# ZenGo-X/zk-paillier

Measured on AMD Instinct MI355X. Metric: RangeProofNi proofs/sec + verifies/sec, n=2048, batch=4096 per GPU (value = verifies/sec; proofs/sec in prove.value), higher is better.
Workload: dtype u32 (29-bit limbs, u64 accumulate)

## Files before the change

zk-paillier_amd/csrc/kernels_basen.hpp:

```cpp
#pragma once
#include "kernels_modexp.hpp"

#define ZKP_UNROLL_STR(x) #x
#define ZKP_UNROLL_(n) _Pragma(ZKP_UNROLL_STR(unroll n))
#define ZKP_UNROLL(n) ZKP_UNROLL_(n)
#ifndef ZKP_BN_ROW_UNROLL
#if ZKP_W == 9
#define ZKP_BN_ROW_UNROLL 8
#else
#define ZKP_BN_ROW_UNROLL 1
#endif
#endif
#ifndef ZKP_BN_ASM
#define ZKP_BN_ASM (ZKP_W == 36)
#endif
namespace zkp {
template <int G> constexpr bool BN_ASM_G = ZKP_BN_ASM && W == 36 && (G == 2 || G == 4);

template <int G> struct BnConst {
  static constexpr int L = Geo<G>::L;
  static constexpr int OFF_MT = 0, OFF_C3 = L, OFF_RRA = 2 * L, OFF_RRB = 3 * L, OFF_N = 4 * L, OFF_R2N = 5 * L, OFF_ONE = 6 * L, OFF_R1A = 7 * L, OFF_R1B = 8 * L, OFF_NI = 9 * L, OFF_OK = 9 * L + 1;
  static constexpr int WORDS = 9 * L + 4;
  static constexpr int STRIDE = WORDS + 2 * L;
};
// ... 532 lines not shown
  store_limbs_global<G>(tab, X, g.gl);
  store_limbs_global<G>(tab + L, Y, g.gl);
  bn_stage<G>(g, g.A(), X);
  bn_stage<G>(g, g.B(), Y);
  const int msb = 31 - __clz(CAP);
#pragma unroll 1
  for (int b = msb - 1; b >= 0; b--) {
    bn_square<G>(g, X);
    if ((CAP >> b) & 1) {
      uint32_t A2[W], B2[W];
      bn_product<G>(g, A2, B2, tab, tab + L);
      bn_stage<G>(g, g.A(), A2);
      bn_stage<G>(g, g.B(), B2);
#pragma unroll
      for (int k = 0; k < W; k++) X[k] = A2[k];
    }
  }
  lds_load_block(Y, g.B() + g.gl * BLK);
  store_limbs_global<G>(out + BC::OFF_RRA, X, g.gl);
  store_limbs_global<G>(out + BC::OFF_RRB, Y, g.gl);
  store_limbs_global<G>(out + BC::OFF_R1A, OA, g.gl);
  store_limbs_global<G>(out + BC::OFF_R1B, OB, g.gl);
  if (g.gl == 0) {
    out[BC::OFF_OK] = ok ? 1u : 0u;
    if (!ok) atomicAnd(all_ok, 0u);
  }
  if (tag && up_tag && gid == 0 && g.gl == 0) {
    tag[1] = up_tag[5];
    __threadfence();
    tag[0] = (ok && up_tag[0] == SETUP_TAG_MAGIC) ? SETUP_TAG_MAGIC : 0u;
  }
}

template <int GS>
__global__ void __launch_bounds__(256, ZKP_WPE) k_expected(EncArgs a, uint32_t* __restrict__ expected, const uint32_t* __restrict__ bn_ok) {
  using CL = ConstLayout<GS>;
  using LL = LdsLayout<GS>;
  if (!*bn_ok) return;
  extern __shared__ __align__(16) uint32_t lds_raw[];
  Grp<GS> g;
  grp_init<GS>(g, lds_raw);
  const int kw = a.n_bits / 32;
  const uint64_t count = a.count_ptr ? (uint64_t)*a.count_ptr : a.count;
  const uint64_t stride = (uint64_t)gridDim.x * LL::GROUPS_PER_BLOCK;
  const uint64_t rounds = (count + stride - 1) / stride;
  const uint32_t* cst = a.consts;
  load_modulus_consts<GS>(g, cst);
  for (uint64_t rd = 0; rd < rounds; rd++) {
    const uint64_t idx = rd * stride + (uint64_t)blockIdx.x * LL::GROUPS_PER_BLOCK + (threadIdx.x / GS);
    const bool live = idx < count;
    const uint64_t item = live ? idx : count - 1;
    uint64_t b;
    bool mask_row;
    const uint32_t* pexp;
    if (a.mode == 2) { b = item; mask_row = a.cipher_x != nullptr; pexp = a.c1 + item * 2 * kw; }
    else {
      b = a.item_proof[item];
      const uint32_t rw = a.item_row[item];
      const uint64_t row = b * a.ef + (rw >> 1);
      mask_row = a.resp_kind[row] != 0;
      const bool use_c1 = mask_row ? (a.resp_j[row] == 1) : !(rw & 1);
      pexp = (use_c1 ? a.c1 : a.c2) + row * 2 * kw;
    }
    if (a.const_stride) {
      const uint64_t i0 = (a.mode == 0 && a.half && item >= a.half) ? item - a.half : item;
      cst = a.consts + (a.mode == 1 ? b : i0 / a.items_per_key) * a.const_stride;
      load_modulus_consts<GS>(g, cst);
    }
    const bool valid = cst[CL::OFF_ST] == 0;
    uint32_t A[W], R[W], Y[W];
    load_value<GS>(g, A, pexp, valid ? 2 * kw : 0);
    stage_const<GS>(g, cst + CL::OFF_R2);
    mm<GS>(g, R, A);
    {
      uint32_t t[W];
      load_value<GS>(g, t, a.cipher_x + b * 2 * kw, (mask_row && valid) ? 2 * kw : 0);
      if (!mask_row && valid && g.gl == 0) t[0] = 1;
      stageB<GS>(g, t);
    }
    mm<GS>(g, Y, R);
    stage_const<GS>(g, cst + CL::OFF_R2);
    mm<GS>(g, R, Y);
    stage_one<GS>(g);
    mm<GS>(g, Y, R);
    canonical_words<GS>(g, Y, cst + CL::OFF_N);
    if (live && mask_row) for (int w = g.gl; w < 2 * kw; w += GS) expected[item * 2 * kw + w] = g.words()[w];
  }
}

struct BnItem {
  const uint32_t* pm; const uint32_t* pr; const uint32_t* pexp; uint32_t* pout;
  uint64_t b; int mw, rw; bool mask_row;
};
__device__ __forceinline__ BnItem bn_item(const EncArgs& a, uint64_t item, const uint32_t* expected) {
  BnItem it{};
  const int kw = a.n_bits / 32;
  it.mw = kw; it.rw = kw;
  if (a.mode == 0) {
    const bool second = a.half && item >= a.half;
    const uint64_t i = second ? item - a.half : item;
    it.mw = a.m_words < 0 ? 0 : (a.m_words ? a.m_words : kw);
    it.rw = a.r_words ? a.r_words : kw;
    it.pm = (second ? a.m2 : a.m) + i * it.mw;
    it.pr = (second ? a.r2 : a.r) + i * it.rw;
    it.pout = (second ? a.out2 : a.out) + i * 2 * kw;
  } else if (a.mode == 2) {
    it.b = item;
    it.pm = a.m + item * kw;
    it.pr = a.r + item * kw;
    it.mask_row = a.cipher_x != nullptr;
    it.pexp = it.mask_row ? expected + item * 2 * kw : a.c1 + item * 2 * kw;
  } else {
    it.b = a.item_proof[item];
    const uint32_t rw = a.item_row[item];
    const uint64_t row = it.b * a.ef + (rw >> 1);
    it.mask_row = a.resp_kind[row] != 0;
    const bool second = (rw & 1) != 0;
    it.pm = (second ? a.resp_w2 : a.resp_w1) + row * kw;
    it.pr = (second ? a.resp_r2 : a.resp_r1) + row * kw;
// ... 568 lines not shown
```

zk-paillier_amd/csrc/kernels_modexp.hpp:

```cpp
#pragma once
#include "../../include/zkp_hip.h"
#include "bigint29.hpp"

namespace zkp {

#ifndef ZKP_WIN
#define ZKP_WIN 5
#endif
#ifndef ZKP_SWIN
#define ZKP_SWIN 6
#endif
#ifndef ZKP_WIN_KEY
#define ZKP_WIN_KEY 6
#endif
constexpr int WIN = ZKP_WIN;
constexpr int WIN_KEY = ZKP_WIN_KEY;
constexpr int SWIN = ZKP_SWIN;
constexpr int TABS = 1 << (SWIN - 1);
constexpr int cmax(int a, int b) { return a > b ? a : b; }
constexpr int TAB = cmax(cmax(1 << WIN, 1 << WIN_KEY), TABS);
static_assert(TABS <= 32 && WIN >= 2 && WIN <= 7 && WIN_KEY >= 2 && WIN_KEY <= 7, "window widths");

template <int G> struct ConstLayout {
  static constexpr int L = Geo<G>::L;
// ... 70 lines not shown
}

template <int G, class LL> __device__ __forceinline__ void mm(const Grp<G, LL>& g, uint32_t (&R)[W], const uint32_t (&A)[W]) {
  montmul<G, false, true>(R, A, g.B(), g.N, g.n1, g.gl);
}
template <int G, class LL> __device__ __forceinline__ void fetch_words(const Grp<G, LL>& g, uint32_t* dst, const uint32_t* src, int nwords) {
  constexpr int NW = LL::NW;
  wave_lds_fence();
  for (int w = g.gl; w < NW + 8; w += G) dst[w] = (w < nwords) ? src[w] : 0u;
  wave_lds_fence();
}

template <int G, class LL> __device__ __forceinline__ void load_value(const Grp<G, LL>& g, uint32_t (&v)[W], const uint32_t* src, int nwords) {
  fetch_words<G>(g, g.words(), src, nwords);
  limbs_from_words(v, g.words(), g.gl);
}

template <int G, class LL> __device__ __forceinline__ void canonical_limbs(const Grp<G, LL>& g, uint32_t (&x)[W]) {
  normalize_exact<G>(x, g.gl);
  bool eq = true;
#pragma unroll
  for (int k = 0; k < W; k++) eq = eq && (x[k] == g.N[k]);
  const unsigned long long m = __ballot(eq);
  const int lane = threadIdx.x & 63;
  const unsigned long long gm = (G == 64) ? ~0ull : (((1ull << G) - 1) << (lane & ~(G - 1)));
  if ((m & gm) == gm) {
#pragma unroll
    for (int k = 0; k < W; k++) x[k] = 0;
  }
}
template <int G, class LL> __device__ __forceinline__ void canonical_words(const Grp<G, LL>& g, uint32_t (&x)[W], const uint32_t* ) {
  canonical_limbs<G>(g, x);
  words_from_limbs<G, LL::NW>(g.words(), g.scr(), x, g.gl);
}


template <int G, bool SAFE, bool TWO = false, int SCHED_FENCE = 0, class LL> __device__ __forceinline__ void mmo_ip(const Grp<G, LL>& g, const uint32_t (&NT)[W], uint32_t (&X)[W]) {
  if constexpr (TWO) montmul2<G>(X, X, g.B(), NT, g.gl);
  else montmul<G, true, SAFE, SCHED_FENCE>(X, X, g.B(), NT, 1u, g.gl);
}
#ifndef ZKP_SQR
#define ZKP_SQR 1
#endif

template <bool SAFE, bool TWO> constexpr bool ladder_squares() { return ZKP_SQR && !SAFE; }
template <int G, bool TWO = false, class LL> __device__ __forceinline__ void msq_ip(const Grp<G, LL>& g, const uint32_t (&NT)[W], uint32_t (&X)[W]) {
  if constexpr (TWO) montsqr2<G>(X, g.B(), NT, g.gl);
  else montsqr<G>(X, g.B(), NT, g.gl);
}

template <int G> __device__ __forceinline__ int wave_exponent_bits(const uint32_t* lw, int exp_bits) {
  int top = (exp_bits >> 5) - 1;
  while (top > 0 && lw[top] == 0) top--;
  int bl = lw[top] ? 32 * top + 32 - __clz(lw[top]) : 0;
#pragma unroll
  for (int off = 32; off >= G && off >= 1; off >>= 1) { const int o = __shfl_xor(bl, off); bl = o > bl ? o : bl; }
  return __builtin_amdgcn_readfirstlane(bl);
}

template <int G, bool SAFE, bool TWO = false, int WIN = zkp::WIN, class LL>
__device__ __forceinline__ void powm_fixed(const Grp<G, LL>& g, uint32_t (&X)[W], int exp_bits, uint32_t* tab, const uint32_t* cst,
                                           const uint32_t* __restrict__ ew ) {
  using CL = ConstLayout<G>;
  constexpr int L = Geo<G>::L;
  constexpr int TABF = 1 << WIN;
  uint32_t NT[W];
// ... 668 lines not shown
```

zk-paillier_amd/csrc/kernels_proofs.hpp:

```cpp
#pragma once
#include "kernels_modexp.hpp"
#include "kernels_gcd.hpp"
#include "sha256_dev.hpp"

namespace zkp {

__device__ __forceinline__ int cmp_words(const uint32_t* a, const uint32_t* b, int n) {
  for (int i = n - 1; i >= 0; i--) {
    const uint32_t x = a[i], y = b[i];
    if (x != y) return x > y ? 1 : -1;
  }
  return 0;
}

__device__ __forceinline__ int challenge_bit(const uint8_t* e, uint32_t i) { return (e[i >> 3] >> (7 - (i & 7))) & 1; }

struct RangeHashArgs {
  const uint32_t* n; uint64_t n_stride;
  const uint32_t* c1; const uint32_t* c2; const uint32_t* range;
  uint32_t kw, ef; uint64_t batch;
  uint8_t* e;
  uint8_t* e_len;
  uint32_t* third;
  uint32_t* two_thirds;
// ... 243 lines not shown
  const uint8_t* db = reinterpret_cast<const uint8_t*>(s.row);
  int lead = 0;
  while (lead < 31 && db[lead] == 0) lead++;
  uint8_t* e = a.e + b * 32;
  for (int i = 0; i < 32; i++) e[i] = (i + lead < 32) ? db[i + lead] : 0;
  const int elen = 32 - lead;
  a.e_len[b] = (uint8_t)elen;
  a.verdict[b] = ((uint32_t)elen * 8 >= a.ef) ? a.ok_value : (uint8_t)ZKP_VERDICT_MALFORMED;
  if (!a.range) return;
  const uint32_t* rg = a.range + b * a.kw;
  uint32_t* t1 = a.third + b * a.kw;
  uint32_t* t2 = a.two_thirds + b * a.kw;
  uint64_t rem = 0;
  for (int w = (int)a.kw - 1; w >= 0; w--) {
    const uint64_t cur = (rem << 32) | rg[w];
    t1[w] = (uint32_t)(cur / 3);
    rem = cur % 3;
  }
  uint32_t carry = 0;
  for (uint32_t w = 0; w < a.kw; w++) { const uint32_t v = t1[w]; t2[w] = (v << 1) | carry; carry = v >> 31; }
}

#ifndef ZKP_TEMPLATE_KERNELS_ONLY
__global__ void __launch_bounds__(64) k_range_hash_wave(RangeHashArgs a) { range_hash_wave_body(a, (int)threadIdx.x, blockIdx.x); }
#endif

struct VerifyPlanArgs {
  const uint8_t* e; const uint8_t* resp_kind;
  const uint32_t* resp_w1; const uint32_t* resp_w2;
  const uint32_t* third; const uint32_t* two_thirds;
  uint32_t kw, ef; uint64_t batch;
  uint8_t* verdict;
  uint32_t* item_proof; uint32_t* item_row; unsigned long long* counter;
};

#ifndef ZKP_TEMPLATE_KERNELS_ONLY
__global__ void __launch_bounds__(256) k_verify_plan(VerifyPlanArgs a) {
  const uint64_t t = (uint64_t)blockIdx.x * 256 + threadIdx.x;
  const bool in = t < a.batch * a.ef;
  uint32_t nitems = 0;
  uint64_t b = 0; uint32_t i = 0;
  if (in && !a.e) {
    b = t / a.ef; i = (uint32_t)(t % a.ef);
    const int kind = a.resp_kind[t];
    nitems = kind == ZKP_RESP_OPEN ? 2 : kind == ZKP_RESP_MASK ? 1 : 0;
  } else if (in) {
    b = t / a.ef; i = (uint32_t)(t % a.ef);
    if (a.verdict[b] != ZKP_VERDICT_MALFORMED) {
      const int ei = challenge_bit(a.e + b * 32, i);
      const int kind = a.resp_kind[t];
      const uint32_t* T1 = a.third + b * a.kw;
      const uint32_t* T2 = a.two_thirds + b * a.kw;
      const uint32_t* w1 = a.resp_w1 + t * a.kw;
      if (!ei && kind == ZKP_RESP_OPEN) {
        const uint32_t* w2 = a.resp_w2 + t * a.kw;
        const int w1_T1 = cmp_words(w1, T1, a.kw), w2_T1 = cmp_words(w2, T1, a.kw);
        const bool flag = (w2_T1 < 0 && w1_T1 > 0 && cmp_words(w1, T2, a.kw) < 0) ||
                          (w1_T1 < 0 && w2_T1 > 0 && cmp_words(w2, T2, a.kw) < 0);
        if (!flag) a.verdict[b] = ZKP_VERDICT_REJECT;
        nitems = 2;
      } else if (ei && kind == ZKP_RESP_MASK) {
        if (cmp_words(w1, T1, a.kw) < 0 || cmp_words(w1, T2, a.kw) > 0) a.verdict[b] = ZKP_VERDICT_REJECT;
        nitems = 1;
      } else {
        a.verdict[b] = ZKP_VERDICT_REJECT;
      }
    }
  }
  if (!a.item_proof) return;
  const unsigned long long m2 = __ballot(nitems == 2), m1 = __ballot(nitems == 1);
  const int lane = threadIdx.x & 63;
  const unsigned long long lt = (1ull << lane) - 1;
  const uint32_t before = 2 * __popcll(m2 & lt) + __popcll(m1 & lt);
  const uint32_t total = 2 * __popcll(m2) + __popcll(m1);
  unsigned long long base = 0;
  if (lane == 0 && total) base = atomicAdd(a.counter, (unsigned long long)total);
  base = __shfl(base, 0);
  for (uint32_t k = 0; k < nitems; k++) {
    a.item_proof[base + before + k] = (uint32_t)b;
    a.item_row[base + before + k] = (i << 1) | k;
  }
}
#endif

struct VerdictMergeArgs {
  uint8_t* verdict; const uint8_t* enc_verdict; const uint8_t* e; const uint8_t* resp_kind; uint32_t ef; uint64_t batch;
};
#ifndef ZKP_TEMPLATE_KERNELS_ONLY
__global__ void __launch_bounds__(256) k_verdict_merge(VerdictMergeArgs a) {
  const uint64_t b = (uint64_t)blockIdx.x * 256 + threadIdx.x;
  if (b >= a.batch) return;
  const uint8_t v = a.verdict[b], ev = a.enc_verdict[b];
  if (v == ZKP_VERDICT_MALFORMED || ev == ZKP_VERDICT_ACCEPT) return;
  if (ev == ZKP_VERDICT_REJECT) { a.verdict[b] = ZKP_VERDICT_REJECT; return; }
  bool any = false;
  for (uint32_t i = 0; i < a.ef; i++) {
    const int ei = challenge_bit(a.e + b * 32, i), kind = a.resp_kind[b * a.ef + i];
    any = any || (!ei && kind == ZKP_RESP_OPEN) || (ei && kind == ZKP_RESP_MASK);
  }
  if (any) a.verdict[b] = ZKP_VERDICT_MALFORMED;
}
#endif

struct ResponseArgs {
  const uint32_t* consts; uint64_t const_stride;
  const uint32_t* x; const uint32_t* r;
  const uint32_t* w1; const uint32_t* w2; const uint32_t* r1; const uint32_t* r2;
  const uint8_t* e; const uint32_t* third; const uint32_t* two_thirds;
  uint8_t* resp_kind; uint8_t* resp_j; uint32_t* resp_w1; uint32_t* resp_r1; uint32_t* resp_w2; uint32_t* resp_r2;
  uint8_t* status;
  uint32_t kw, ef; uint64_t batch;
};

template <int G>
// ... 456 lines not shown
```

zk-paillier_amd/csrc/zkp_api.hip:

```cpp
#include <hip/hip_runtime.h>
#include <dlfcn.h>

#include <algorithm>
#include <cstdio>
#include <cstdlib>
#include <new>
#include <cstring>
#include <exception>
#include <mutex>
#include <string>
#include <thread>
#include <type_traits>
#include <vector>

#include "../../include/zkp_hip.h"
#include "../../include/zkp_hip_diag.h"
#include "kernels_modexp.hpp"
#include "kernels_proofs.hpp"
#include "kernels_inv.hpp"
#include "kernels_serde.hpp"
#include "kernels_serde_write.hpp"
#include "kernels_serde_scan.hpp"
#include "kernels_sample.hpp"
#include "kernels_coprime.hpp"
#if ZKP_W == 36 || ZKP_W == 18 || ZKP_W == 9
#define ZKP_HAS_BASEN 1
#include "kernels_basen.hpp"
#ifndef ZKP_R2L5_ITEMS_PER_CU
#define ZKP_R2L5_ITEMS_PER_CU 1ull
#endif
#include "kernels_basen_r2l.hpp"
#else
#define ZKP_HAS_BASEN 0
#endif

using namespace zkp;

struct DevBuf {
  void* p = nullptr;
  size_t cap = 0;
  uint32_t* tag = nullptr;
  uint64_t gen = 0, tag_gen = 0;
};

struct StageBlock { void* p; size_t cap; };

enum ScratchSlot : int {
  S_E = 0,
  S_ELEN = 1,
  S_T1 = 2, S_T2 = 3,
  S_IPROOF = 4, S_IROW = 5, S_COUNTER = 6,
  S_STATUS = 7,
  S_MGF = 8, S_PRIMES = 9,
  S_DLOG_E = 10,
  S_TMP1 = 11, S_TMP2 = 12, S_TMP3 = 13,
  S_SCHED = 15,
  S_TMP4 = 16, S_TMP5 = 17,
  S_WORK_COUNTER = 18,
  S_ENCV = 19,
  S_MP_NN = 20, S_MP_INVST = 21,
  S_MP_T0 = 22,
  S_MP_END = 32,
  S_CM_SUM = 34, S_CM_FLAGS = 35,
  S_CM_T0 = 36,
  S_CM_END = 44,
  S_SAMPLE_THIRD = 44, S_SAMPLE_META = 45, S_SAMPLE_STATUS = 46,
  S_RESIDUE = 47,
  S_COUNT = 48
};
static_assert(S_MP_T0 + 9 < S_MP_END && S_MP_END <= S_CM_SUM && S_CM_T0 + 7 < S_CM_END && S_CM_END <= S_SAMPLE_THIRD && S_RESIDUE < S_COUNT,
              "scratch slot runs overlap");

struct zkp_ctx {
  std::vector<StageBlock> stage_free;
  std::vector<std::pair<void*, size_t>> last_wiped;
  uint32_t* setup_flag = nullptr;
  uint32_t* setup_flag_host = nullptr;
  int device = 0;
  hipStream_t stream = nullptr;
  bool owns_stream = true;
  int cus = 0;
  const struct LatEngine* eng[2] = {nullptr, nullptr};
  zkp_ctx* eng_ctx[2] = {nullptr, nullptr};
  const struct LatEngine* lat = nullptr;
  zkp_ctx* lat_ctx = nullptr;
  int geometry = 0;
  int last_geometry = 0;
  hipStream_t side = nullptr;
  hipEvent_t ev_fork = nullptr, ev_join = nullptr;
  bool side_busy = false;
  hipStream_t copy = nullptr;
  std::vector<hipEvent_t> ev_pipe;
  bool copy_busy = false;
  int last_host_blocks = 0;
  uint64_t scan_fast = 0, scan_fallback = 0;
  hipEvent_t ev_scan[5] = {nullptr, nullptr, nullptr, nullptr, nullptr};
  int scan_phases = 0;
  zkp_ctx* split_ctx = nullptr;
  hipStream_t split_stream = nullptr;
  hipEvent_t ev_split[2] = {nullptr, nullptr};
  int split_calls = 1;
  int last_split = 0;
  int key_cache = 1;
  int host_chunks = -1;
  std::string err;
  DevBuf consts, consts2, table, scratch[S_COUNT];
  DevBuf bn_ncst, bn_consts, bn_table, bn_expected, bn_raw, bn_left;
  int enc_form = ZKP_ENC_FORM_AUTO;
  int bn_occ[2][2] = {{0, 0}, {0, 0}};
  int bn_last_g = 0;
  bool bn_last_per_key = false;
  bool bn_last_r2l = false;
  int bn_r2l_lanes = 0;
  int bn_last_r2l_lanes = 0;
  int bn_r2l = 1;
  const RangeHashArgs* fuse_hash = nullptr;
  bool fuse_hash_taken = false;
  int fuse_hash_on = 1;
  int grid_expected = 1;
  DevBuf bn_flag;
  bool timing = false;
  std::vector<std::pair<hipEvent_t, hipEvent_t>> ev;
  size_t ev_used = 0;
  uint64_t timed_launches = 0, timed_modexps = 0;
  static constexpr size_t PINNED_SLOTS = 4096;
  unsigned long long* pinned_counts = nullptr;
  size_t pinned_used = 0;
};

#define HIPCHK(ctx, call)                                                                         \
  do {                                                                                            \
    hipError_t e_ = (call);                                                                       \
    if (e_ != hipSuccess) {                                                                       \
      (ctx)->err = std::string(#call) + ": " + hipGetErrorString(e_);                             \
      return e_ == hipErrorOutOfMemory ? ZKP_ENOMEM : ZKP_EDEVICE;                                \
    }                                                                                             \
  } while (0)

static int32_t zkp_caught(zkp_ctx* c, int32_t st, const char* what) noexcept {
  if (c) { try { c->err = what; } catch (...) {} }
// ... 390 lines not shown
  HIPCHK(c, hipEventCreateWithFlags(&c->ev_fork, hipEventDisableTiming));
  HIPCHK(c, hipEventCreateWithFlags(&c->ev_join, hipEventDisableTiming));
  HIPCHK(c, hipStreamCreateWithFlags(&c->side, hipStreamNonBlocking));
  return ZKP_OK;
}

template <int G, class K> static int32_t table_for(zkp_ctx* c, K kernel, uint64_t items, unsigned* blocks_out) {
  using LL = LdsLayout<G>;
  const uint64_t need = (items + LL::GROUPS_PER_BLOCK - 1) / LL::GROUPS_PER_BLOCK;
  const unsigned blocks = (unsigned)std::max<uint64_t>(1, std::min<uint64_t>(need, (uint64_t)resident_blocks<G>(c, kernel)));
  *blocks_out = blocks;
  return ensure(c, c->table, (size_t)blocks * LL::GROUPS_PER_BLOCK * TAB * Geo<G>::L * sizeof(uint32_t));
}

constexpr bool PAIR_LADDER_BUILD = ZKP_W <= 9;
template <int G> static bool pair_ladder(const zkp_ctx* c, uint64_t items) {
  if (c->enc_form == ZKP_ENC_FORM_ALWAYS) return false;
  if constexpr (PAIR_LADDER_BUILD && 2 * G <= 64) return items * 2 * G <= 4ull * (uint64_t)c->cus * 64;
  (void)c; (void)items;
  return false;
}

#if ZKP_HAS_BASEN
constexpr int BN_GA = 72 / W, BN_GB = 144 / W;
#ifdef ZKP_SPLIT_TU
extern template __global__ void zkp::k_enc_basen<BN_GA>(EncArgs, const uint32_t*, uint32_t*, uint32_t*);
extern template __global__ void zkp::k_enc_basen<BN_GB>(EncArgs, const uint32_t*, uint32_t*, uint32_t*);
extern template __global__ void zkp::k_enc_basen_keys<BN_GA>(EncArgs, const uint32_t*, const uint32_t*, uint32_t*, uint32_t*);
extern template __global__ void zkp::k_enc_basen_keys<BN_GB>(EncArgs, const uint32_t*, const uint32_t*, uint32_t*, uint32_t*);
extern template __global__ void zkp::k_basen_finish<BN_GA>(EncArgs, const uint32_t*, const uint32_t*, int, const uint32_t*, const uint32_t*, const uint32_t*);
extern template __global__ void zkp::k_basen_finish<BN_GB>(EncArgs, const uint32_t*, const uint32_t*, int, const uint32_t*, const uint32_t*, const uint32_t*);
extern template __global__ void zkp::k_setup_basen<BN_GA>(const uint32_t*, uint32_t*, uint64_t, uint32_t*, const uint32_t*, uint32_t*);
extern template __global__ void zkp::k_setup_basen<BN_GB>(const uint32_t*, uint32_t*, uint64_t, uint32_t*, const uint32_t*, uint32_t*);
extern template __global__ void zkp::k_expected<2 * BN_GA>(EncArgs, uint32_t*, const uint32_t*);
extern template __global__ void zkp::k_expected<2 * BN_GB>(EncArgs, uint32_t*, const uint32_t*);
extern template __global__ void zkp::k_diag_basen<BN_GA>(const uint32_t*, int, const uint32_t*, const uint32_t*, const uint32_t*, const uint32_t*, uint32_t*, uint32_t*);
extern template __global__ void zkp::k_diag_basen<BN_GB>(const uint32_t*, int, const uint32_t*, const uint32_t*, const uint32_t*, const uint32_t*, uint32_t*, uint32_t*);
#endif
constexpr size_t BASEN_DIAG_LDS = 4096;
static int enc_form_from_env() {
  const char* e = std::getenv("ZKP_BASEN");
  if (e && e[0] == '0') return ZKP_ENC_FORM_N2;
  if (e && e[0] == 's') return ZKP_ENC_FORM_SHARED;
  if (e && e[0] == 'a') return ZKP_ENC_FORM_ALWAYS;
  return ZKP_ENC_FORM_AUTO;
}
template <int G> static int32_t basen_prepare(zkp_ctx* c, const uint32_t* n, uint64_t n_stride, uint64_t nkeys, uint32_t n_bits) {
  int32_t st = run_setup<G>(c, n, n_stride, (int)(n_bits / 32), 0, nkeys, c->bn_ncst);
  if (st) return st;
  if ((st = ensure(c, c->bn_consts, (size_t)(nkeys + 1) * BnConst<G>::STRIDE * sizeof(uint32_t)))) return st;
  HIPCHK(c, hipMemsetAsync((char*)c->bn_consts.p + (size_t)nkeys * BnConst<G>::STRIDE * sizeof(uint32_t), 0, BnConst<G>::STRIDE * sizeof(uint32_t), c->stream));
  if ((st = ensure(c, c->bn_flag, 64))) return st;
  HIPCHK(c, hipMemsetD32Async((hipDeviceptr_t)c->bn_flag.p, 1, 2, c->stream));
  constexpr unsigned GPB = 64 / G;
  uint32_t* tag = nullptr;
  if ((st = setup_tag(c, c->bn_consts, nkeys, &tag))) return st;
  hipLaunchKernelGGL(k_setup_basen<G>, dim3((unsigned)((nkeys + GPB - 1) / GPB)), dim3(64), GPB * BN_SETUP_LDS_WORDS * sizeof(uint32_t), c->stream,
                     (const uint32_t*)c->bn_ncst.p, (uint32_t*)c->bn_consts.p, nkeys, (uint32_t*)c->bn_flag.p, tag ? (const uint32_t*)c->bn_ncst.tag : nullptr, tag);
  HIPCHK(c, hipGetLastError());
  return ZKP_OK;
}
static bool r2l_one_per_simd(const zkp_ctx* c, uint64_t count, bool listed, uint64_t hashes) {
  const uint64_t simds = 4ull * (uint64_t)c->cus;
  const uint64_t expect = (listed && c->grid_expected) ? expected_items(count) : count;
  return hashes < simds && expect + hashes <= simds;
}
template <int GS> static bool launch_basen(zkp_ctx* c, const EncArgs& a_in, EncArgs* rest) {
  if constexpr (GS != 2 * BN_GA && GS != 2 * BN_GB) { (void)c; (void)a_in; (void)rest; return false; }
// ... 24 lines not shown
    }
    auto give_up = [&]() { c->err.clear(); *rest = a_in; return false; };
    if (basen_prepare<G>(c, a.n, a.n_stride, nkeys, (uint32_t)a.n_bits)) return give_up();
    int& per_cu = c->bn_occ[per_key ? 1 : 0][G == BN_GB ? 1 : 0];
    if (!per_cu) {
      const hipError_t e = per_key ? hipOccupancyMaxActiveBlocksPerMultiprocessor(&per_cu, k_enc_basen_keys<G>, 256, BL::BYTES_PER_BLOCK)
                                   : hipOccupancyMaxActiveBlocksPerMultiprocessor(&per_cu, k_enc_basen<G>, 256, BL::BYTES_PER_BLOCK);
      if (e != hipSuccess || per_cu < 1) per_cu = 1;
    }
    const uint64_t need = (a.count + BL::GROUPS_PER_BLOCK - 1) / BL::GROUPS_PER_BLOCK;
    uint64_t grid = std::min<uint64_t>(need, (uint64_t)per_cu * c->cus);
    if (a.count_ptr && a.mode == 1 && c->grid_expected) {
      const uint64_t need_e = (expected_items(a.count) + BL::GROUPS_PER_BLOCK - 1) / BL::GROUPS_PER_BLOCK;
      const uint64_t per_cu_e = (need_e + (uint64_t)c->cus - 1) / (uint64_t)c->cus;
      grid = std::min<uint64_t>(grid, per_cu_e * (uint64_t)c->cus);
    }
    const unsigned blocks = (unsigned)std::max<uint64_t>(1, grid);
    const size_t entries = per_key ? BN_KEYS_TAB_ENTRIES : BN_TAB_ENTRIES;
    if (!r2l_launch && ensure(c, c->bn_table, (size_t)blocks * BL::GROUPS_PER_BLOCK * entries * 2 * Geo<G>::L * sizeof(uint32_t))) return give_up();
    if (ensure(c, c->bn_raw, (size_t)a.count * 2 * Geo<G>::L * sizeof(uint32_t))) return give_up();
    const uint32_t* ok = per_key ? (const uint32_t*)c->bn_flag.p + 1 : (const uint32_t*)c->bn_consts.p + BnConst<G>::OFF_OK;
    if (per_key) {
      if (ensure(c, c->bn_left, 16 + (size_t)a.count * sizeof(uint32_t))) return give_up();
      if (hipMemsetAsync(c->bn_left.p, 0, 16, c->stream) != hipSuccess) return give_up();
      a.left_count = (unsigned long long*)c->bn_left.p;
      a.left_list = (uint32_t*)((char*)c->bn_left.p + 16);
      rest->remap = a.left_list; rest->remap_count = a.left_count;
      rest->work_counter = a.work_counter + 1;
    }
    const bool products = a.mode == 1 || (a.mode == 2 && a.cipher_x);
    if (products) {
      if (ensure(c, c->bn_expected, (size_t)a.count * 2 * kw * sizeof(uint32_t))) return give_up();
      using LS = LdsLayout<GS>;
      const uint64_t eneed = (a.count + LS::GROUPS_PER_BLOCK - 1) / LS::GROUPS_PER_BLOCK;
      const unsigned eblocks = (unsigned)std::max<uint64_t>(1, std::min<uint64_t>(eneed, 2ull * c->cus));
      hipLaunchKernelGGL(k_expected<GS>, dim3(eblocks), dim3(256), LS::BYTES_PER_BLOCK, c->stream, a, (uint32_t*)c->bn_expected.p, ok);
    }
    c->bn_last_g = G; c->bn_last_per_key = per_key; c->bn_last_r2l = r2l_launch;
#if ZKP_W == 9
    if (r2l_launch) {
      if constexpr (G == 8) {
        const unsigned waves = (unsigned)std::max<uint64_t>(1, std::min<uint64_t>(a.count, r2l_items < a.count ? std::max<uint64_t>(r2l_items, 2ull * 4 * (uint64_t)c->cus) : 8ull * 4 * (uint64_t)c->cus));
        const int lanes = c->bn_r2l_lanes ? c->bn_r2l_lanes : (a.count <= ZKP_R2L5_ITEMS_PER_CU * (uint64_t)c->cus ? 36 : 12);
        c->bn_last_r2l_lanes = lanes;
        if (lanes == 36) {
          RangeHashArgs h{};
          uint64_t enc_wgs = std::max<uint64_t>(1, std::min<uint64_t>(a.count, 4ull * (uint64_t)c->cus));
          size_t dyn = 0;
          if (c->fuse_hash && c->fuse_hash->batch < (uint64_t)c->cus) {
            h = *c->fuse_hash;
            c->fuse_hash_taken = true;
            enc_wgs = std::max<uint64_t>(1, std::min<uint64_t>(enc_wgs, (uint64_t)c->cus - h.batch));
            dyn = (size_t)hw_lds_words((int)h.kw) * sizeof(uint32_t);
          }
          hipLaunchKernelGGL(k_enc_basen_r2l5, dim3((unsigned)(h.batch + enc_wgs)), dim3(320), dyn, c->stream, a, (const uint32_t*)c->bn_consts.p, (uint32_t*)c->bn_raw.p, h);
        }
        else {
          RangeHashArgs h{};
          uint64_t enc_wgs = waves;
          size_t dyn = 0;
          const uint64_t simds = 4ull * (uint64_t)c->cus;
          const uint64_t hashes = c->fuse_hash ? c->fuse_hash->batch : 0;
          if (r2l_one_per_simd(c, a.count, a.count_ptr != nullptr, hashes)) {
            enc_wgs = std::max<uint64_t>(1, std::min<uint64_t>(enc_wgs, simds - hashes));
            if (c->fuse_hash) {
              h = *c->fuse_hash;
              h.wave_blocks = HW_BLOCKS;
              c->fuse_hash_taken = true;
              dyn = (size_t)hw_lds_words<HW_BLOCKS>((int)h.kw) * sizeof(uint32_t);
// ... 101 lines not shown
#endif
  *out = c;
  return ZKP_OK;
}

extern "C" int32_t zkp_ctx_create(int32_t device_id, zkp_ctx** out) try {
  return ctx_create(device_id, nullptr, true, out);
} ZKP_CATCH(nullptr)

extern "C" int32_t zkp_ctx_create_on_stream(int32_t device_id, void* hip_stream, zkp_ctx** out) try {
  return ctx_create(device_id, (hipStream_t)hip_stream, false, out);
} ZKP_CATCH(nullptr)

extern "C" int32_t zkp_ctx_set_geometry(zkp_ctx* c, int32_t limbs_per_lane) try {
  if (!c) return ZKP_EINVAL;
  if (limbs_per_lane != 0 && limbs_per_lane != W && engine_with(c, limbs_per_lane) < 0) {
    c->err = "zkp_ctx_set_geometry: no engine with " + std::to_string(limbs_per_lane) + " limbs per lane is loaded";
    return ZKP_EINVAL;
  }
  c->geometry = limbs_per_lane;
  return ZKP_OK;
} ZKP_CATCH(c)
extern "C" int32_t zkp_ctx_last_geometry(zkp_ctx* c) { return c ? c->last_geometry : 0; }
extern "C" int32_t zkp_ctx_latency_limbs_per_lane(zkp_ctx* c) { return (c && c->eng[0]) ? c->eng[0]->limbs_per_lane : 0; }

extern "C" int32_t zkp_ctx_destroy(zkp_ctx* c) try {
  if (!c) return ZKP_EINVAL;
  (void)hipSetDevice(c->device);
  (void)hipStreamSynchronize(c->stream);
  if (c->split_ctx) { (void)hipStreamSynchronize(c->split_stream); (void)c->eng[0]->p_zkp_ctx_destroy(c->split_ctx); }
  if (c->split_stream) (void)hipStreamDestroy(c->split_stream);
  for (hipEvent_t e : c->ev_split) if (e) (void)hipEventDestroy(e);
  for (int k = 0; k < 2; k++) if (c->eng_ctx[k]) (void)c->eng[k]->p_zkp_ctx_destroy(c->eng_ctx[k]);
  for (DevBuf* b : {&c->consts, &c->consts2, &c->table, &c->bn_ncst, &c->bn_consts, &c->bn_table, &c->bn_expected, &c->bn_raw, &c->bn_flag, &c->bn_left}) { if (b->p) (void)hipFree(b->p); if (b->tag) (void)hipFree(b->tag); }
  for (auto& b : c->scratch) if (b.p) (void)hipFree(b.p);
  for (auto& e : c->ev) { (void)hipEventDestroy(e.first); (void)hipEventDestroy(e.second); }
  if (c->pinned_counts) (void)hipHostFree(c->pinned_counts);
  for (auto& b : c->stage_free) (void)hipFree(b.p);
  if (c->setup_flag) (void)hipFree(c->setup_flag);
  if (c->setup_flag_host) (void)hipHostFree(c->setup_flag_host);
  if (c->side) { (void)hipStreamSynchronize(c->side); (void)hipStreamDestroy(c->side); }
  if (c->copy) { (void)hipStreamSynchronize(c->copy); (void)hipStreamDestroy(c->copy); }
  for (hipEvent_t e : c->ev_pipe) (void)hipEventDestroy(e);
  for (hipEvent_t e : c->ev_scan) if (e) (void)hipEventDestroy(e);
  if (c->ev_fork) (void)hipEventDestroy(c->ev_fork);
  if (c->ev_join) (void)hipEventDestroy(c->ev_join);
  if (c->owns_stream && c->stream) (void)hipStreamDestroy(c->stream);
  delete c;
  return ZKP_OK;
} ZKP_CATCH(c)

extern "C" int32_t zkp_ctx_release_staging(zkp_ctx* c) try {
  if (!c) return ZKP_EINVAL;
  HIPCHK(c, hipSetDevice(c->device));
  HIPCHK(c, hipStreamSynchronize(c->stream));
  for (auto& b : c->stage_free) (void)hipFree(b.p);
  c->stage_free.clear();
  c->last_wiped.clear();
  for (DevBuf* b : {&c->bn_table, &c->bn_raw, &c->bn_expected}) { if (b->p) (void)hipFree(b->p); b->p = nullptr; b->cap = 0; }
  if (c->split_ctx) (void)c->eng[0]->p_zkp_ctx_release_staging(c->split_ctx);
  for (int k = 0; k < 2; k++)
    if (c->eng_ctx[k]) { const int32_t st = c->eng[k]->p_zkp_ctx_release_staging(c->eng_ctx[k]); if (st) { c->err = c->eng[k]->p_zkp_last_error_string(c->eng_ctx[k]); return st; } }
  return ZKP_OK;
} ZKP_CATCH(c)

extern "C" const char* zkp_backend_name(void) { return "hip-gfx950"; }
extern "C" int32_t zkp_build_limbs_per_lane(void) { return W; }
// ... 461 lines not shown
```

zk-paillier_amd/csrc/zkp_api_proofs.inc:

```

enum : unsigned { RA_RANGE = 1, RA_CIPHERTEXT = 2, RA_PAIRS = 4, RA_RESP = 8 };
static bool range_args_ok(const zkp_range_ni_proofs* p, unsigned need = RA_RANGE | RA_CIPHERTEXT | RA_PAIRS | RA_RESP) {
  if (!p) return false;
  if (p->n_bits != 1024 && p->n_bits != 2048 && p->n_bits != 4096) return false;
  if (p->batch > (1ull << 24) || p->error_factor > 256) return false;
  if (p->n_stride != 0 && p->n_stride != p->n_bits / 32) return false;
  if (p->batch == 0) return true;
  if (!p->n || ((need & RA_RANGE) && !p->range) || ((need & RA_CIPHERTEXT) && !p->ciphertext)) return false;
  if (p->error_factor && (need & RA_PAIRS) && (!p->c1 || !p->c2)) return false;
  if (p->error_factor && (need & RA_RESP) && (!p->resp_kind || !p->resp_j || !p->resp_w1 || !p->resp_r1 || !p->resp_w2 || !p->resp_r2)) return false;
  return true;
}

static zkp_range_ni_proofs range_slice(const zkp_range_ni_proofs& p, size_t EF, uint64_t lo, uint64_t count) {
  const size_t kw = p.n_bits / 32;
  zkp_range_ni_proofs q = p;
  q.batch = count;
  if (q.n) q.n += lo * p.n_stride;
  if (q.range) q.range += lo * kw;
  if (q.ciphertext) q.ciphertext += lo * 2 * kw;
  for (uint32_t** a : {&q.c1, &q.c2}) if (*a) *a += lo * EF * 2 * kw;
  for (uint8_t** a : {&q.resp_kind, &q.resp_j}) if (*a) *a += lo * EF;
  for (uint32_t** a : {&q.resp_w1, &q.resp_r1, &q.resp_w2, &q.resp_r2}) if (*a) *a += lo * EF * kw;
  return q;
// ... 436 lines not shown
                                 const uint8_t* e_len_in = nullptr) {
  using CL = ConstLayout<G>;
  const uint32_t kw = p.n_bits / 32, EF = p.error_factor;
  const uint64_t nkeys = p.n_stride ? p.batch : 1, rows = p.batch * EF;
  int32_t st;
  if ((st = run_setup<G>(c, p.n, p.n_stride, (int)kw, 1, nkeys, c->consts))) return st;
  if ((st = ensure(c, c->scratch[S_E], p.batch * 32))) return st;
  if ((st = ensure(c, c->scratch[S_ELEN], p.batch))) return st;
  const uint64_t enc_blocks = (2 * rows + LdsLayout<G>::GROUPS_PER_BLOCK - 1) / LdsLayout<G>::GROUPS_PER_BLOCK;
  const char* two_env = std::getenv("ZKP_TWO_STREAMS");
  const uint64_t cus = (uint64_t)c->cus;
  const bool two_rule = W == 36 ? (enc_blocks <= 3 * cus / 2 || enc_blocks >= 12 * cus) : W == 9 ? enc_blocks <= 5 * cus / 2 : enc_blocks <= 11 * cus / 4;
  const bool two = rows != 0 && !e_in && (two_env ? two_env[0] == '1' : two_rule);
  const bool fuse = two && c->fuse_hash_on && p.batch < cus && basen_r2l_takes_hashes<G>(c, p.n_stride, p.n_bits, 2 * rows, p.batch);
  hipStream_t hs = c->stream;
  uint8_t* enc_verdict = verdict;
  if (two) {
    if ((st = ensure(c, c->scratch[S_ENCV], p.batch))) return st;
    enc_verdict = (uint8_t*)c->scratch[S_ENCV].p;
    HIPCHK(c, hipMemsetAsync(enc_verdict, ZKP_VERDICT_ACCEPT, p.batch, c->stream));
  }
  if (two && !fuse) {
    if ((st = side_stream(c))) return st;
    HIPCHK(c, hipEventRecord(c->ev_fork, c->stream));
    HIPCHK(c, hipStreamWaitEvent(c->side, c->ev_fork, 0));
    c->side_busy = true;
    hs = c->side;
  }
  RangeHashArgs fused_hash{};
  if ((st = range_hash<G>(c, p, (uint8_t*)c->scratch[S_E].p, (uint8_t*)c->scratch[S_ELEN].p, verdict, ZKP_VERDICT_ACCEPT, e_in, e_len_in, hs, fuse ? &fused_hash : nullptr))) return st;
  if (rows == 0) return ZKP_OK;
  if ((st = ensure(c, c->scratch[S_IPROOF], 2 * rows * 4))) return st;
  if ((st = ensure(c, c->scratch[S_IROW], 2 * rows * 4))) return st;
  if ((st = ensure(c, c->scratch[S_COUNTER], 16))) return st;
  HIPCHK(c, hipMemsetAsync(c->scratch[S_COUNTER].p, 0, 16, c->stream));
  VerifyPlanArgs v{(const uint8_t*)c->scratch[S_E].p, p.resp_kind, p.resp_w1, p.resp_w2, (const uint32_t*)c->scratch[S_T1].p,
                   (const uint32_t*)c->scratch[S_T2].p, kw, EF, p.batch, verdict, (uint32_t*)c->scratch[S_IPROOF].p,
                   (uint32_t*)c->scratch[S_IROW].p, (unsigned long long*)c->scratch[S_COUNTER].p};
  const dim3 plan_grid((unsigned)((rows + 255) / 256));
  VerifyPlanArgs pred = v; pred.item_proof = nullptr; pred.item_row = nullptr; pred.counter = nullptr;
  if (two) {
    if (!fuse) {
      hipLaunchKernelGGL(k_verify_plan, plan_grid, dim3(256), 0, c->side, pred);
      HIPCHK(c, hipGetLastError());
      HIPCHK(c, hipEventRecord(c->ev_join, c->side));
    }
    VerifyPlanArgs list = v; list.e = nullptr; list.verdict = nullptr;
    hipLaunchKernelGGL(k_verify_plan, plan_grid, dim3(256), 0, c->stream, list);
  } else {
    hipLaunchKernelGGL(k_verify_plan, plan_grid, dim3(256), 0, c->stream, v);
  }
  HIPCHK(c, hipGetLastError());
  unsigned blocks = 0;
  if ((st = table_for<G>(c, k_enc<G, true>, 2 * rows, &blocks))) return st;
  EncArgs a{};
  a.n = p.n; a.n_stride = p.n_stride; a.consts = (const uint32_t*)c->consts.p; a.const_stride = p.n_stride ? (uint64_t)CL::WORDS : 0;
  a.table = (uint32_t*)c->table.p; a.count = 2 * rows ; a.n_bits = (int)p.n_bits; a.mode = 1;
  a.item_proof = (const uint32_t*)c->scratch[S_IPROOF].p; a.item_row = (const uint32_t*)c->scratch[S_IROW].p;
  a.resp_w1 = p.resp_w1; a.resp_r1 = p.resp_r1; a.resp_w2 = p.resp_w2; a.resp_r2 = p.resp_r2; a.resp_kind = p.resp_kind; a.resp_j = p.resp_j;
  a.c1 = p.c1; a.c2 = p.c2; a.cipher_x = p.ciphertext; a.verdict = enc_verdict;
  a.count_ptr = (const unsigned long long*)c->scratch[S_COUNTER].p; a.ef = EF;
  if (p.n_stride == 0 && !pair_ladder<G>(c, a.count) && (st = build_schedule(c, p.n, p.n_bits, &a.sched))) return st;
  if ((st = fresh_work_counter(c, &a.work_counter))) return st;
  {
    TimedRegion tr(c, 0);
    FuseHashScope fh(c, fuse ? &fused_hash : nullptr);
    launch_k_enc<G>(c, blocks, a);
  }
  HIPCHK(c, hipGetLastError());
  if (fuse) {
    if (!c->fuse_hash_taken) {
// ... 478 lines not shown
```

zk-paillier_amd/csrc/zkp_kernels_basen.hip:

```cpp
#define ZKP_TEMPLATE_KERNELS_ONLY
#include "../../include/zkp_hip.h"
#include "kernels_basen.hpp"

namespace zkp {
constexpr int BN_GA = 72 / W, BN_GB = 144 / W;
template __global__ void k_enc_basen<BN_GA>(EncArgs, const uint32_t*, uint32_t*, uint32_t*);
template __global__ void k_enc_basen<BN_GB>(EncArgs, const uint32_t*, uint32_t*, uint32_t*);
template __global__ void k_enc_basen_keys<BN_GA>(EncArgs, const uint32_t*, const uint32_t*, uint32_t*, uint32_t*);
template __global__ void k_enc_basen_keys<BN_GB>(EncArgs, const uint32_t*, const uint32_t*, uint32_t*, uint32_t*);
template __global__ void k_basen_finish<BN_GA>(EncArgs, const uint32_t*, const uint32_t*, int, const uint32_t*, const uint32_t*, const uint32_t*);
template __global__ void k_basen_finish<BN_GB>(EncArgs, const uint32_t*, const uint32_t*, int, const uint32_t*, const uint32_t*, const uint32_t*);
template __global__ void k_setup_basen<BN_GA>(const uint32_t*, uint32_t*, uint64_t, uint32_t*, const uint32_t*, uint32_t*);
template __global__ void k_setup_basen<BN_GB>(const uint32_t*, uint32_t*, uint64_t, uint32_t*, const uint32_t*, uint32_t*);
template __global__ void k_expected<2 * BN_GA>(EncArgs, uint32_t*, const uint32_t*);
template __global__ void k_expected<2 * BN_GB>(EncArgs, uint32_t*, const uint32_t*);
template __global__ void k_diag_basen<BN_GA>(const uint32_t*, int, const uint32_t*, const uint32_t*, const uint32_t*, const uint32_t*, uint32_t*, uint32_t*);
template __global__ void k_diag_basen<BN_GB>(const uint32_t*, int, const uint32_t*, const uint32_t*, const uint32_t*, const uint32_t*, uint32_t*, uint32_t*);
}
```

Before: 3438.

## Precompute per-proof Montgomery x once and compact expected-product work to masked rows

Adds a kernel that converts each proof's cipher_x into Montgomery form once per batch, so the expected-value kernel no longer repeats that conversion for every row. The verify planner now also builds a compacted list of masked items, so k_expected only processes rows whose product is actually needed. The per-item chain of four Montgomery multiplies is reduced to one multiply plus a single conditional subtraction. The expected kernel's grid is sized from measured occupancy instead of a fixed multiple of CUs. This costs an extra launch, an extra buffer and an extra atomic counter, and it relies on the shortened reduction being exact.

```diff
diff --git a/zk-paillier_amd/csrc/kernels_basen.hpp b/zk-paillier_amd/csrc/kernels_basen.hpp
--- a/zk-paillier_amd/csrc/kernels_basen.hpp
+++ b/zk-paillier_amd/csrc/kernels_basen.hpp
@@ -588,8 +588,11 @@
   }
 }
 
+__device__ __forceinline__ const uint32_t* expected_consts(const EncArgs& a, uint64_t b) {
+  return a.consts + (a.const_stride ? (a.mode == 1 ? b : b / a.items_per_key) * a.const_stride : 0);
+}
 template <int GS>
-__global__ void __launch_bounds__(256, ZKP_WPE) k_expected(EncArgs a, uint32_t* __restrict__ expected, const uint32_t* __restrict__ bn_ok) {
+__global__ void __launch_bounds__(256, ZKP_WPE) k_expected_x(EncArgs a, uint64_t batch, uint32_t* __restrict__ xr, const uint32_t* __restrict__ bn_ok) {
   using CL = ConstLayout<GS>;
   using LL = LdsLayout<GS>;
   if (!*bn_ok) return;
@@ -597,7 +600,34 @@
   Grp<GS> g;
   grp_init<GS>(g, lds_raw);
   const int kw = a.n_bits / 32;
-  const uint64_t count = a.count_ptr ? (uint64_t)*a.count_ptr : a.count;
+  const uint64_t stride = (uint64_t)gridDim.x * LL::GROUPS_PER_BLOCK;
+  const uint64_t rounds = (batch + stride - 1) / stride;
+  for (uint64_t rd = 0; rd < rounds; rd++) {
+    const uint64_t gid = rd * stride + (uint64_t)blockIdx.x * LL::GROUPS_PER_BLOCK + (threadIdx.x / GS);
+    const bool live = gid < batch;
+    const uint64_t b = live ? gid : batch - 1;
+    const uint32_t* cst = expected_consts(a, b);
+    load_modulus_consts<GS>(g, cst);
+    const bool valid = cst[CL::OFF_ST] == 0;
+    uint32_t A[W], R[W];
+    load_value<GS>(g, A, a.cipher_x + b * 2 * kw, valid ? 2 * kw : 0);
+    stage_const<GS>(g, cst + CL::OFF_R2);
+    mm<GS>(g, R, A);
+    if (live) store_limbs_global<GS>(xr + b * Geo<GS>::L, R, g.gl);
+  }
+}
+template <int GS>
+__global__ void __launch_bounds__(256, ZKP_WPE) k_expected(EncArgs a, uint32_t* __restrict__ expected, const uint32_t* __restrict__ bn_ok,
+                                                           const uint32_t* __restrict__ mask_item, const unsigned long long* __restrict__ mask_count,
+                                                           const uint32_t* __restrict__ xr) {
+  using CL = ConstLayout<GS>;
+  using LL = LdsLayout<GS>;
+  if (!*bn_ok) return;
+  extern __shared__ __align__(16) uint32_t lds_raw[];
+  Grp<GS> g;
+  grp_init<GS>(g, lds_raw);
+  const int kw = a.n_bits / 32;
+  const uint64_t count = a.mode == 2 ? a.count : (uint64_t)*mask_count;
   const uint64_t stride = (uint64_t)gridDim.x * LL::GROUPS_PER_BLOCK;
   const uint64_t rounds = (count + stride - 1) / stride;
   const uint32_t* cst = a.consts;
@@ -605,42 +635,28 @@
   for (uint64_t rd = 0; rd < rounds; rd++) {
     const uint64_t idx = rd * stride + (uint64_t)blockIdx.x * LL::GROUPS_PER_BLOCK + (threadIdx.x / GS);
     const bool live = idx < count;
-    const uint64_t item = live ? idx : count - 1;
-    uint64_t b;
-    bool mask_row;
+    const uint64_t at = live ? idx : count - 1;
+    uint64_t item, b;
     const uint32_t* pexp;
-    if (a.mode == 2) { b = item; mask_row = a.cipher_x != nullptr; pexp = a.c1 + item * 2 * kw; }
+    if (a.mode == 2) { item = at; b = item; pexp = a.c1 + item * 2 * kw; }
     else {
+      item = mask_item[at];
       b = a.item_proof[item];
-      const uint32_t rw = a.item_row[item];
-      const uint64_t row = b * a.ef + (rw >> 1);
-      mask_row = a.resp_kind[row] != 0;
-      const bool use_c1 = mask_row ? (a.resp_j[row] == 1) : !(rw & 1);
-      pexp = (use_c1 ? a.c1 : a.c2) + row * 2 * kw;
+      const uint64_t row = b * a.ef + (a.item_row[item] >> 1);
+      pexp = (a.resp_j[row] == 1 ? a.c1 : a.c2) + row * 2 * kw;
     }
     if (a.const_stride) {
-      const uint64_t i0 = (a.mode == 0 && a.half && item >= a.half) ? item - a.half : item;
-      cst = a.consts + (a.mode == 1 ? b : i0 / a.items_per_key) * a.const_stride;
+      cst = expected_consts(a, b);
       load_modulus_consts<GS>(g, cst);
     }
     const bool valid = cst[CL::OFF_ST] == 0;
-    uint32_t A[W], R[W], Y[W];
+    uint32_t A[W], Y[W];
     load_value<GS>(g, A, pexp, valid ? 2 * kw : 0);
-    stage_const<GS>(g, cst + CL::OFF_R2);
-    mm<GS>(g, R, A);
-    {
-      uint32_t t[W];
-      load_value<GS>(g, t, a.cipher_x + b * 2 * kw, (mask_row && valid) ? 2 * kw : 0);
-      if (!mask_row && valid && g.gl == 0) t[0] = 1;
-      stageB<GS>(g, t);
-    }
-    mm<GS>(g, Y, R);
-    stage_const<GS>(g, cst + CL::OFF_R2);
-    mm<GS>(g, R, Y);
-    stage_one<GS>(g);
-    mm<GS>(g, Y, R);
-    canonical_words<GS>(g, Y, cst + CL::OFF_N);
-    if (live && mask_row) for (int w = g.gl; w < 2 * kw; w += GS) expected[item * 2 * kw + w] = g.words()[w];
+    stage_const<GS>(g, xr + b * Geo<GS>::L);
+    mm<GS>(g, Y, A);
+    reduce_once<GS>(g, Y);
+    words_from_limbs<GS, LL::NW>(g.words(), g.scr(), Y, g.gl);
+    if (live) for (int w = g.gl; w < 2 * kw; w += GS) expected[item * 2 * kw + w] = g.words()[w];
   }
 }
 
diff --git a/zk-paillier_amd/csrc/kernels_modexp.hpp b/zk-paillier_amd/csrc/kernels_modexp.hpp
--- a/zk-paillier_amd/csrc/kernels_modexp.hpp
+++ b/zk-paillier_amd/csrc/kernels_modexp.hpp
@@ -126,6 +126,22 @@
 template <int G, class LL> __device__ __forceinline__ void canonical_words(const Grp<G, LL>& g, uint32_t (&x)[W], const uint32_t* ) {
   canonical_limbs<G>(g, x);
   words_from_limbs<G, LL::NW>(g.words(), g.scr(), x, g.gl);
+}
+
+template <int G, class LL> __device__ __forceinline__ void reduce_once(const Grp<G, LL>& g, uint32_t (&x)[W]) {
+  normalize_exact<G>(x, g.gl);
+  int cmp = 0;
+#pragma unroll
+  for (int k = 0; k < W; k++) cmp = x[k] != g.N[k] ? (x[k] > g.N[k] ? 1 : -1) : cmp;
+  const int lane = threadIdx.x & 63;
+  const unsigned long long gm = (G == 64) ? ~0ull : (((1ull << G) - 1) << (lane & ~(G - 1)));
+  const unsigned long long gt = __ballot(cmp > 0) & gm, lt = __ballot(cmp < 0) & gm;
+  if (gt >= lt) {
+#pragma unroll
+    for (int k = 0; k < W; k++) x[k] += LMASK - g.N[k];
+    if (g.gl == 0) x[0] += 1;
+  }
+  normalize_exact<G>(x, g.gl);
 }
 
 
diff --git a/zk-paillier_amd/csrc/kernels_proofs.hpp b/zk-paillier_amd/csrc/kernels_proofs.hpp
--- a/zk-paillier_amd/csrc/kernels_proofs.hpp
+++ b/zk-paillier_amd/csrc/kernels_proofs.hpp
@@ -299,6 +299,7 @@
   uint32_t kw, ef; uint64_t batch;
   uint8_t* verdict;
   uint32_t* item_proof; uint32_t* item_row; unsigned long long* counter;
+  uint32_t* mask_item; unsigned long long* mask_counter;
 };
 
 #ifndef ZKP_TEMPLATE_KERNELS_ONLY
@@ -347,6 +348,12 @@
     a.item_proof[base + before + k] = (uint32_t)b;
     a.item_row[base + before + k] = (i << 1) | k;
   }
+  if (!a.mask_item) return;
+  const uint32_t mtotal = __popcll(m1);
+  unsigned long long mbase = 0;
+  if (lane == 0 && mtotal) mbase = atomicAdd(a.mask_counter, (unsigned long long)mtotal);
+  mbase = __shfl(mbase, 0);
+  if (nitems == 1) a.mask_item[mbase + __popcll(m1 & lt)] = (uint32_t)(base + before);
 }
 #endif
 
diff --git a/zk-paillier_amd/csrc/zkp_api.hip b/zk-paillier_amd/csrc/zkp_api.hip
--- a/zk-paillier_amd/csrc/zkp_api.hip
+++ b/zk-paillier_amd/csrc/zkp_api.hip
@@ -54,6 +54,7 @@
   S_MGF = 8, S_PRIMES = 9,
   S_DLOG_E = 10,
   S_TMP1 = 11, S_TMP2 = 12, S_TMP3 = 13,
+  S_IMASK = 14,
   S_SCHED = 15,
   S_TMP4 = 16, S_TMP5 = 17,
   S_WORK_COUNTER = 18,
@@ -106,6 +107,8 @@
   std::string err;
   DevBuf consts, consts2, table, scratch[S_COUNT];
   DevBuf bn_ncst, bn_consts, bn_table, bn_expected, bn_raw, bn_left;
+  DevBuf bn_xr;
+  int bn_exp_occ[2] = {0, 0};
   int enc_form = ZKP_ENC_FORM_AUTO;
   int bn_occ[2][2] = {{0, 0}, {0, 0}};
   int bn_last_g = 0;
@@ -562,8 +565,10 @@
 extern template __global__ void zkp::k_basen_finish<BN_GB>(EncArgs, const uint32_t*, const uint32_t*, int, const uint32_t*, const uint32_t*, const uint32_t*);
 extern template __global__ void zkp::k_setup_basen<BN_GA>(const uint32_t*, uint32_t*, uint64_t, uint32_t*, const uint32_t*, uint32_t*);
 extern template __global__ void zkp::k_setup_basen<BN_GB>(const uint32_t*, uint32_t*, uint64_t, uint32_t*, const uint32_t*, uint32_t*);
-extern template __global__ void zkp::k_expected<2 * BN_GA>(EncArgs, uint32_t*, const uint32_t*);
-extern template __global__ void zkp::k_expected<2 * BN_GB>(EncArgs, uint32_t*, const uint32_t*);
+extern template __global__ void zkp::k_expected<2 * BN_GA>(EncArgs, uint32_t*, const uint32_t*, const uint32_t*, const unsigned long long*, const uint32_t*);
+extern template __global__ void zkp::k_expected<2 * BN_GB>(EncArgs, uint32_t*, const uint32_t*, const uint32_t*, const unsigned long long*, const uint32_t*);
+extern template __global__ void zkp::k_expected_x<2 * BN_GA>(EncArgs, uint64_t, uint32_t*, const uint32_t*);
+extern template __global__ void zkp::k_expected_x<2 * BN_GB>(EncArgs, uint64_t, uint32_t*, const uint32_t*);
 extern template __global__ void zkp::k_diag_basen<BN_GA>(const uint32_t*, int, const uint32_t*, const uint32_t*, const uint32_t*, const uint32_t*, uint32_t*, uint32_t*);
 extern template __global__ void zkp::k_diag_basen<BN_GB>(const uint32_t*, int, const uint32_t*, const uint32_t*, const uint32_t*, const uint32_t*, uint32_t*, uint32_t*);
 #endif
@@ -654,9 +659,17 @@
     if (products) {
       if (ensure(c, c->bn_expected, (size_t)a.count * 2 * kw * sizeof(uint32_t))) return give_up();
       using LS = LdsLayout<GS>;
+      const uint64_t batch = a.mode == 1 ? a.count / (2 * (uint64_t)a.ef) : a.count;
+      if (ensure(c, c->bn_xr, (size_t)batch * Geo<GS>::L * sizeof(uint32_t))) return give_up();
+      hipLaunchKernelGGL(k_expected_x<GS>, dim3((unsigned)((batch + LS::GROUPS_PER_BLOCK - 1) / LS::GROUPS_PER_BLOCK)), dim3(256), LS::BYTES_PER_BLOCK, c->stream, a, batch,
+                         (uint32_t*)c->bn_xr.p, ok);
+      int& eocc = c->bn_exp_occ[G == BN_GB ? 1 : 0];
+      if (!eocc) eocc = resident_blocks<GS>(c, k_expected<GS>);
       const uint64_t eneed = (a.count + LS::GROUPS_PER_BLOCK - 1) / LS::GROUPS_PER_BLOCK;
-      const unsigned eblocks = (unsigned)std::max<uint64_t>(1, std::min<uint64_t>(eneed, 2ull * c->cus));
-      hipLaunchKernelGGL(k_expected<GS>, dim3(eblocks), dim3(256), LS::BYTES_PER_BLOCK, c->stream, a, (uint32_t*)c->bn_expected.p, ok);
+      const unsigned eblocks = (unsigned)std::max<uint64_t>(1, std::min<uint64_t>(eneed, (uint64_t)eocc));
+      hipLaunchKernelGGL(k_expected<GS>, dim3(eblocks), dim3(256), LS::BYTES_PER_BLOCK, c->stream, a, (uint32_t*)c->bn_expected.p, ok,
+                         a.mode == 1 ? (const uint32_t*)c->scratch[S_IMASK].p : nullptr,
+                         a.mode == 1 ? (const unsigned long long*)c->scratch[S_COUNTER].p + 1 : nullptr, (const uint32_t*)c->bn_xr.p);
     }
     c->bn_last_g = G; c->bn_last_per_key = per_key; c->bn_last_r2l = r2l_launch;
 #if ZKP_W == 9
@@ -824,7 +837,7 @@
   if (c->split_stream) (void)hipStreamDestroy(c->split_stream);
   for (hipEvent_t e : c->ev_split) if (e) (void)hipEventDestroy(e);
   for (int k = 0; k < 2; k++) if (c->eng_ctx[k]) (void)c->eng[k]->p_zkp_ctx_destroy(c->eng_ctx[k]);
-  for (DevBuf* b : {&c->consts, &c->consts2, &c->table, &c->bn_ncst, &c->bn_consts, &c->bn_table, &c->bn_expected, &c->bn_raw, &c->bn_flag, &c->bn_left}) { if (b->p) (void)hipFree(b->p); if (b->tag) (void)hipFree(b->tag); }
+  for (DevBuf* b : {&c->consts, &c->consts2, &c->table, &c->bn_ncst, &c->bn_consts, &c->bn_table, &c->bn_expected, &c->bn_raw, &c->bn_flag, &c->bn_left, &c->bn_xr}) { if (b->p) (void)hipFree(b->p); if (b->tag) (void)hipFree(b->tag); }
   for (auto& b : c->scratch) if (b.p) (void)hipFree(b.p);
   for (auto& e : c->ev) { (void)hipEventDestroy(e.first); (void)hipEventDestroy(e.second); }
   if (c->pinned_counts) (void)hipHostFree(c->pinned_counts);
diff --git a/zk-paillier_amd/csrc/zkp_api_proofs.inc b/zk-paillier_amd/csrc/zkp_api_proofs.inc
--- a/zk-paillier_amd/csrc/zkp_api_proofs.inc
+++ b/zk-paillier_amd/csrc/zkp_api_proofs.inc
@@ -492,11 +492,13 @@
   if (rows == 0) return ZKP_OK;
   if ((st = ensure(c, c->scratch[S_IPROOF], 2 * rows * 4))) return st;
   if ((st = ensure(c, c->scratch[S_IROW], 2 * rows * 4))) return st;
+  if ((st = ensure(c, c->scratch[S_IMASK], 2 * rows * 4))) return st;
   if ((st = ensure(c, c->scratch[S_COUNTER], 16))) return st;
   HIPCHK(c, hipMemsetAsync(c->scratch[S_COUNTER].p, 0, 16, c->stream));
   VerifyPlanArgs v{(const uint8_t*)c->scratch[S_E].p, p.resp_kind, p.resp_w1, p.resp_w2, (const uint32_t*)c->scratch[S_T1].p,
                    (const uint32_t*)c->scratch[S_T2].p, kw, EF, p.batch, verdict, (uint32_t*)c->scratch[S_IPROOF].p,
-                   (uint32_t*)c->scratch[S_IROW].p, (unsigned long long*)c->scratch[S_COUNTER].p};
+                   (uint32_t*)c->scratch[S_IROW].p, (unsigned long long*)c->scratch[S_COUNTER].p,
+                   (uint32_t*)c->scratch[S_IMASK].p, (unsigned long long*)c->scratch[S_COUNTER].p + 1};
   const dim3 plan_grid((unsigned)((rows + 255) / 256));
   VerifyPlanArgs pred = v; pred.item_proof = nullptr; pred.item_row = nullptr; pred.counter = nullptr;
   if (two) {
diff --git a/zk-paillier_amd/csrc/zkp_kernels_basen.hip b/zk-paillier_amd/csrc/zkp_kernels_basen.hip
--- a/zk-paillier_amd/csrc/zkp_kernels_basen.hip
+++ b/zk-paillier_amd/csrc/zkp_kernels_basen.hip
@@ -12,8 +12,10 @@
 template __global__ void k_basen_finish<BN_GB>(EncArgs, const uint32_t*, const uint32_t*, int, const uint32_t*, const uint32_t*, const uint32_t*);
 template __global__ void k_setup_basen<BN_GA>(const uint32_t*, uint32_t*, uint64_t, uint32_t*, const uint32_t*, uint32_t*);
 template __global__ void k_setup_basen<BN_GB>(const uint32_t*, uint32_t*, uint64_t, uint32_t*, const uint32_t*, uint32_t*);
-template __global__ void k_expected<2 * BN_GA>(EncArgs, uint32_t*, const uint32_t*);
-template __global__ void k_expected<2 * BN_GB>(EncArgs, uint32_t*, const uint32_t*);
+template __global__ void k_expected<2 * BN_GA>(EncArgs, uint32_t*, const uint32_t*, const uint32_t*, const unsigned long long*, const uint32_t*);
+template __global__ void k_expected<2 * BN_GB>(EncArgs, uint32_t*, const uint32_t*, const uint32_t*, const unsigned long long*, const uint32_t*);
+template __global__ void k_expected_x<2 * BN_GA>(EncArgs, uint64_t, uint32_t*, const uint32_t*);
+template __global__ void k_expected_x<2 * BN_GB>(EncArgs, uint64_t, uint32_t*, const uint32_t*);
 template __global__ void k_diag_basen<BN_GA>(const uint32_t*, int, const uint32_t*, const uint32_t*, const uint32_t*, const uint32_t*, uint32_t*, uint32_t*);
 template __global__ void k_diag_basen<BN_GB>(const uint32_t*, int, const uint32_t*, const uint32_t*, const uint32_t*, const uint32_t*, uint32_t*, uint32_t*);
 }
```

Result: no change. 3408 (-0.9%).
